# leonzheng2/Safe-Exploration-with-Simulator-in-RL-algorithms

Hardware: AMD Instinct MI355X
Metric: env-steps/sec (higher is better)
Workload: dtype f64; 1 GPU; ARS V2 iteration, 3-segment swimmer, 512 directions/GPU x 2 rollouts x H=1000 (BASELINE configs[2] per GPU); directions_total=512, directions_per_gpu=512, horizon=1000, segments=3, trajectory_capture=True, full_covariance=True, parallelism=directions sharded over 1 GPU(s), 1 all-gather/iteration, ranks_seen=1

## Files before the change

### include/swimmer_hip.h

```cpp
#ifndef SWIMMER_HIP_H
#define SWIMMER_HIP_H

#include <stdint.h>

#ifdef __cplusplus
extern "C" {
#endif

#define SW_ABI_VERSION 3
#define SW_MAX_SEGMENTS 8

#define SW_OK 0
#define SW_ERR_NULL 1
#define SW_ERR_SEGMENTS 2
#define SW_ERR_SIZE 3
#define SW_ERR_PARAM 4
#define SW_ERR_LAUNCH 5

#define SW_STATUS_OK 0
#define SW_STATUS_SINGULAR 1
#define SW_STATUS_NONFINITE 2
#define SW_STATUS_RANGE 4
#define SW_STATUS_PARAM 8

#define SW_FLAG_ROLLOUT_LANE 1
#define SW_FLAG_ROLLOUT_QUAD 2

#define SW_FLAG_MODEL_TWIN 4

typedef struct sw_params {
    int32_t n;
    int32_t flags;
    double l_i;
    double m_i;
    double k;
    double h;
    double dir_x;
    double dir_y;
} sw_params;

int sw_abi_version(void);
const char *sw_strerror(int code);
int sw_max_segments(void);

int sw_reset_f64(const sw_params *p, int64_t n_env, double *state, void *stream);

int sw_step_f64(const sw_params *p, int64_t n_env, const double *state_in,
                const double *action, double *state_out, double *reward,
                int32_t *status, void *stream);

int sw_step_residual_f64(const sw_params *p, int64_t n_env, const double *state, const double *action,
                         const double *next_ref, double *partial, void *stream);
int64_t sw_step_residual_blocks(int64_t n_env);

int sw_step_residual_pop_f64(const sw_params *base, int64_t n_cand, const double *cand, int64_t n_env,
                             const double *state, const double *action, const double *next_ref, double *partial,
                             double *value, int32_t *cand_status, void *stream);

int sw_accel_f64(const sw_params *p, int64_t n_env, const double *state,
                 const double *action, double *gdd, double *tdd, void *stream);

int sw_rollout_f64(const sw_params *p, int64_t n_roll, int32_t H, const double *policies,
                   const double *mean, const double *inv_std, const double *state0,
                   double *returns, double *traj, double *final_state, double *moments,
                   int32_t *status, void *stream);

#define SW_COST_ABS_OBS 0
#define SW_COST_MAX_ABS_THETADOT 1
int sw_safe_rollouts_f64(const sw_params *real, const sw_params *sim, int64_t n_roll, int32_t H,
                         const double *policies, int32_t cost_kind, int32_t cost_index, double sim_thresh,
                         double real_thresh, double *returns, double *traj, int32_t *first_refused,
                         int32_t *violations, int32_t *status, void *stream);

int64_t sw_moments_blocks(int64_t n_roll);

int sw_ars_rollouts_f64(const sw_params *p, int64_t dir_begin, int64_t n_dir, int32_t H,
                        const double *policy, const double *deltas, double nu,
                        const double *mean, const double *inv_std, double *returns,
                        double *traj, double *moments, int32_t *status, void *stream);

int sw_ars_gate_f64(const sw_params *sim, int64_t dir_begin, int64_t n_dir, int32_t H,
                    const double *policy, const double *deltas, double nu,
                    const double *mean, const double *inv_std, double sim_thresh,
                    int32_t *admit, double *returns, int32_t *status, void *stream);

int sw_ars_update_f64(const sw_params *p, int64_t n_dir, const double *returns,
                      const double *deltas, double *policy, double alpha, double b,
                      int64_t top_b, const double *moments, int64_t n_moment_rows,
                      double *running, int64_t n_new_states, double *mean, double *inv_std,
                      double *sigma_out, void *stream);

int sw_ars_rollouts_multi_f64(const sw_params *p, int64_t n_agent, int64_t n_dir, int32_t H,
                              const double *policy, const double *deltas, double nu,
                              const double *mean, const double *inv_std, double *returns,
                              double *moments, int32_t *status, void *stream);

int sw_ars_update_multi_f64(const sw_params *p, int64_t n_agent, int64_t n_dir, const double *returns,
                            const double *deltas, double *policy, double alpha, double b,
                            int64_t top_b, const double *moments, int64_t n_moment_rows,
                            double *running, int64_t n_new_states, double *mean, double *inv_std,
                            double *sigma_out, void *stream);

#define SW_CACLA_HIDDEN 12
#define SW_CACLA_NET_DOUBLES(n) (SW_CACLA_HIDDEN * (2 * (n) + 2) + 2 * SW_CACLA_HIDDEN + 1)
int sw_cacla_run_f64(const sw_params *p, int64_t n_agent, int32_t n_iter, int32_t train,
                     const double *gamma, const double *alpha, const double *noise, double *weights,
                     double *state, double *rewards, int32_t *actor_updates, int32_t *status, void *stream);

int sw_ars_update_gathered_f64(const sw_params *p, int64_t n_dir, const double *gathered,
// ... 72 lines not shown
```

### safe-exploration-with-simulator-in-rl-algorithms_amd/_build.py

```python
import os
import shutil
import subprocess
import tempfile
from concurrent.futures import ThreadPoolExecutor

_HERE = os.path.dirname(os.path.abspath(__file__))
CSRC = os.path.join(_HERE, "csrc")
LIB_PATH = os.environ.get("SWIMMER_HIP_LIB") or os.path.join(CSRC, "libswimmer_hip.so")
OBJ_DIR = LIB_PATH + ".obj"
SOURCES = ["swimmer_kernels.hip", "swimmer_abi.hip", "swimmer_cacla.hip", "direct_comm.cpp", "host_rng.cpp"]
FAMILIES = ["swimmer_rollout_row.hip", "swimmer_rollout_n3.hip", "swimmer_rollout_lane.hip", "swimmer_step.hip",
            "swimmer_cov.hip", "swimmer_update.hip"]
HOST_ONLY = {"host_rng.cpp"}
HEADERS = ["rlglue_env.cpp", os.path.join("..", "..", "include", "rlglue_swimmer.h"),
           "swimmer_launch.h", "swimmer_cov.h", "swimmer_device.h", "swimmer_rollout_lane.inc",
           "swimmer_rollout_quad3.inc", "swimmer_rollout_oct3.inc", "swimmer_rollout_row.inc",
           "swimmer_rollout_multi.inc", "swimmer_update.inc", "swimmer_quad3.h",
           "swimmer_oct3.h", "swimmer_row.h", "swimmer_row_fused.h", "swimmer_twin.h",
           os.path.join("..", "..", "include", "swimmer_hip.h")] + FAMILIES
HIPCC_FLAGS = ["-O3", "--offload-arch=gfx950", "-std=c++17", "-fPIC"] + os.environ.get("SWIMMER_HIPCC_EXTRA", "").split()
HOST_FLAGS = ["-O3", "-std=c++17", "-fPIC"]
LINK_LIBS = ["-ldl"]
LLVM = "/opt/rocm/lib/llvm/bin"


def _hipcc():
    exe = shutil.which("hipcc") or "/opt/rocm/bin/hipcc"
    if not os.path.exists(exe):
        raise RuntimeError("hipcc not found: the swimmer HIP library cannot be built")
    return exe


def _newer_than(path, deps):
    if not os.path.exists(path):
        return True
    t = os.path.getmtime(path)
    deps = [os.path.join(CSRC, d) for d in deps]
    return any(os.path.exists(d) and os.path.getmtime(d) > t for d in deps)


def is_stale():
    return _newer_than(LIB_PATH, SOURCES + HEADERS)


RLGLUE_LIB_PATH = os.path.join(CSRC, "librlglue_swimmer_hip.so")


def _object(src):
    return os.path.join(OBJ_DIR, os.path.splitext(src)[0] + ".o")


def _compile(src, verbose):
    flags = HOST_FLAGS + ["-x", "c++"] if src in HOST_ONLY else HIPCC_FLAGS + ["-x", "hip"]
    cmd = [_hipcc()] + flags + ["-c", os.path.join(CSRC, src), "-o", _object(src)]
    if verbose:
        print(" ".join(cmd), flush=True)
    done = subprocess.run(cmd, cwd=CSRC, capture_output=True, text=True)
    if done.returncode != 0:
        raise RuntimeError(f"hipcc failed on {src} (exit {done.returncode}):\n{done.stderr}")
    if verbose and done.stderr:
        print(done.stderr, end="", flush=True)


def build_library(force=False, verbose=False):
    if not force and not is_stale() and os.path.exists(RLGLUE_LIB_PATH):
        return LIB_PATH
    os.makedirs(OBJ_DIR, exist_ok=True)
    todo = [s for s in SOURCES if force or _newer_than(_object(s), [s] + HEADERS)]
    jobs = max(1, min(16, int(os.environ.get("MAX_JOBS", 16))))
    with ThreadPoolExecutor(max_workers=jobs) as pool:
        for _ in pool.map(lambda s: _compile(s, verbose), todo):
            pass
    cmd = ([_hipcc(), "-shared", "-fPIC", "--offload-arch=gfx950"] + [_object(s) for s in SOURCES]
           + LINK_LIBS + ["-o", LIB_PATH])
    if verbose:
        print(" ".join(cmd), flush=True)
    subprocess.check_call(cmd, cwd=CSRC)
    cmd = [_hipcc()] + HIPCC_FLAGS + ["-shared", os.path.join(CSRC, "rlglue_env.cpp"), "-L" + CSRC,
                                      "-lswimmer_hip", "-Wl,-rpath,$ORIGIN", "-o", RLGLUE_LIB_PATH]
    if verbose:
        print(" ".join(cmd), flush=True)
    subprocess.check_call(cmd, cwd=CSRC)
    return LIB_PATH


def disassemble(lib=None, raw_insn=False):
    magic = b"__CLANG_OFFLOAD_BUNDLE__"
    lines = []
    with tempfile.TemporaryDirectory() as tmp:
        fat = os.path.join(tmp, "fat.bin")
        subprocess.run([f"{LLVM}/llvm-objcopy", "-O", "binary", "--only-section=.hip_fatbin", lib or LIB_PATH, fat],
                       check=True)
        with open(fat, "rb") as f:
            blob = f.read()
        starts, at = [], blob.find(magic)
        while at >= 0:
            starts.append(at)
            at = blob.find(magic, at + 1)
        for k, (a, b) in enumerate(zip(starts, starts[1:] + [len(blob)])):
            bundle, elf = os.path.join(tmp, f"bundle{k}.bin"), os.path.join(tmp, f"gfx950_{k}.elf")
# ... 9 lines not shown
```

### safe-exploration-with-simulator-in-rl-algorithms_amd/_lib.py

```python
import ctypes
import os

import numpy as np
import torch

from . import _build

ABI_VERSION = 3
MAX_SEGMENTS = 8

ERR_NAMES = {0: "SW_OK", 1: "SW_ERR_NULL", 2: "SW_ERR_SEGMENTS", 3: "SW_ERR_SIZE",
             4: "SW_ERR_PARAM", 5: "SW_ERR_LAUNCH"}
STATUS_SINGULAR = 1
STATUS_NONFINITE = 2
STATUS_RANGE = 4
FLAG_ROLLOUT_LANE = 1
FLAG_ROLLOUT_QUAD = 2
FLAG_MODEL_TWIN = 4
COST_ABS_OBS = 0
COST_MAX_ABS_THETADOT = 1


class SwParams(ctypes.Structure):
    _fields_ = [("n", ctypes.c_int32), ("flags", ctypes.c_int32), ("l_i", ctypes.c_double),
                ("m_i", ctypes.c_double), ("k", ctypes.c_double), ("h", ctypes.c_double),
                ("dir_x", ctypes.c_double), ("dir_y", ctypes.c_double)]

    @classmethod
    def make(cls, n=3, l_i=1.0, m_i=1.0, k=10.0, h=1e-3, direction=(1.0, 0.0), flags=0):
        return cls(int(n), int(flags), float(l_i), float(m_i), float(k), float(h),
                   float(direction[0]), float(direction[1]))

    @property
    def d(self):
        return 2 * self.n + 2

    @property
    def m(self):
        return self.n - 1


class SwimmerHipError(RuntimeError):
    pass


def kernel_flags(name):
    try:
        return {"auto": 0, "lane": FLAG_ROLLOUT_LANE, "quad": FLAG_ROLLOUT_QUAD}[name]
    except KeyError:
        raise SwimmerHipError(f"rollout kernel must be 'auto', 'lane' or 'quad', not {name!r}")


_lib = None

_PROTOTYPES = {
    "sw_abi_version": (ctypes.c_int, []),
    "sw_max_segments": (ctypes.c_int, []),
    "sw_strerror": (ctypes.c_char_p, [ctypes.c_int]),
    "sw_moments_blocks": (ctypes.c_int64, [ctypes.c_int64]),
    "sw_reset_f64": (ctypes.c_int, [ctypes.c_void_p, ctypes.c_int64, ctypes.c_void_p,
                                    ctypes.c_void_p]),
    "sw_step_f64": (ctypes.c_int, [ctypes.c_void_p, ctypes.c_int64] + [ctypes.c_void_p] * 6),
    "sw_step_residual_f64": (ctypes.c_int, [ctypes.c_void_p, ctypes.c_int64] + [ctypes.c_void_p] * 5),
    "sw_step_residual_blocks": (ctypes.c_int64, [ctypes.c_int64]),
    "sw_step_residual_pop_f64": (ctypes.c_int, [ctypes.c_void_p, ctypes.c_int64, ctypes.c_void_p, ctypes.c_int64]
                                 + [ctypes.c_void_p] * 7),
    "sw_accel_f64": (ctypes.c_int, [ctypes.c_void_p, ctypes.c_int64] + [ctypes.c_void_p] * 5),
    "sw_rollout_f64": (ctypes.c_int, [ctypes.c_void_p, ctypes.c_int64, ctypes.c_int32]
                       + [ctypes.c_void_p] * 10),
    "sw_safe_rollouts_f64": (ctypes.c_int, [ctypes.c_void_p, ctypes.c_void_p, ctypes.c_int64, ctypes.c_int32,
                                            ctypes.c_void_p, ctypes.c_int32, ctypes.c_int32, ctypes.c_double,
                                            ctypes.c_double] + [ctypes.c_void_p] * 6),
    "sw_ars_rollouts_f64": (ctypes.c_int, [ctypes.c_void_p, ctypes.c_int64, ctypes.c_int64,
                                           ctypes.c_int32, ctypes.c_void_p, ctypes.c_void_p,
                                           ctypes.c_double] + [ctypes.c_void_p] * 7),
    "sw_ars_gate_f64": (ctypes.c_int, [ctypes.c_void_p, ctypes.c_int64, ctypes.c_int64, ctypes.c_int32,
                                       ctypes.c_void_p, ctypes.c_void_p, ctypes.c_double, ctypes.c_void_p,
                                       ctypes.c_void_p, ctypes.c_double] + [ctypes.c_void_p] * 4),
    "sw_ars_update_f64": (ctypes.c_int, [ctypes.c_void_p, ctypes.c_int64, ctypes.c_void_p,
                                         ctypes.c_void_p, ctypes.c_void_p, ctypes.c_double,
                                         ctypes.c_double, ctypes.c_int64, ctypes.c_void_p,
                                         ctypes.c_int64, ctypes.c_void_p, ctypes.c_int64,
                                         ctypes.c_void_p, ctypes.c_void_p, ctypes.c_void_p,
                                         ctypes.c_void_p]),
    "sw_ars_rollouts_multi_f64": (ctypes.c_int, [ctypes.c_void_p, ctypes.c_int64, ctypes.c_int64,
                                                 ctypes.c_int32, ctypes.c_void_p, ctypes.c_void_p,
                                                 ctypes.c_double] + [ctypes.c_void_p] * 6),
    "sw_ars_update_multi_f64": (ctypes.c_int, [ctypes.c_void_p, ctypes.c_int64, ctypes.c_int64,
                                               ctypes.c_void_p, ctypes.c_void_p, ctypes.c_void_p,
                                               ctypes.c_double, ctypes.c_double, ctypes.c_int64,
                                               ctypes.c_void_p, ctypes.c_int64, ctypes.c_void_p,
                                               ctypes.c_int64, ctypes.c_void_p, ctypes.c_void_p,
                                               ctypes.c_void_p, ctypes.c_void_p]),
    "sw_cacla_run_f64": (ctypes.c_int, [ctypes.c_void_p, ctypes.c_int64, ctypes.c_int32, ctypes.c_int32]
                         + [ctypes.c_void_p] * 9),
    "sw_traj_moments_f64": (ctypes.c_int, [ctypes.c_void_p, ctypes.c_int64, ctypes.c_int32,
                                           ctypes.c_void_p, ctypes.c_void_p, ctypes.c_void_p]),
    "sw_cov_acc_doubles": (ctypes.c_int64, [ctypes.c_void_p, ctypes.c_int64, ctypes.c_int32]),
    "sw_env1_create": (ctypes.c_int, [ctypes.POINTER(ctypes.c_void_p)]),
    "sw_env1_destroy": (None, [ctypes.c_void_p]),
    "sw_env1_io": (ctypes.POINTER(ctypes.c_double), [ctypes.c_void_p]),
    "sw_env1_step": (ctypes.c_int, [ctypes.c_void_p, ctypes.c_void_p, ctypes.POINTER(ctypes.c_int32)]),
    "sw_env1_accel": (ctypes.c_int, [ctypes.c_void_p, ctypes.c_void_p]),
    "sw_comm_available": (ctypes.c_int, []),
    "sw_comm_unique_id": (ctypes.c_int, [ctypes.c_void_p]),
    "sw_comm_create": (ctypes.c_int, [ctypes.POINTER(ctypes.c_void_p), ctypes.c_void_p, ctypes.c_int32,
                                      ctypes.c_int32]),
    "sw_comm_destroy": (None, [ctypes.c_void_p]),
    "sw_comm_all_gather_f64": (ctypes.c_int, [ctypes.c_void_p, ctypes.c_void_p, ctypes.c_void_p,
                                              ctypes.c_int64, ctypes.c_void_p]),
    "sw_comm_last_error": (ctypes.c_char_p, [ctypes.c_void_p]),
    "sw_issue_probe": (ctypes.c_int, [ctypes.c_int32, ctypes.c_int32, ctypes.c_void_p, ctypes.c_void_p]),
    "sw_issue_probe_grid": (ctypes.c_int, [ctypes.c_int32, ctypes.c_int32, ctypes.c_int32, ctypes.c_int32,
                                           ctypes.c_void_p, ctypes.c_void_p]),
    "sw_mt19937_uniform_pm1": (ctypes.c_int, [ctypes.c_void_p, ctypes.POINTER(ctypes.c_int32),
                                              ctypes.c_int64, ctypes.c_void_p]),
    "sw_mt19937_force_isa": (ctypes.c_int, [ctypes.c_int]),
    "sw_ars_pipeline_create": (ctypes.c_int, [ctypes.POINTER(ctypes.c_void_p)]),
    "sw_ars_pipeline_destroy": (None, [ctypes.c_void_p]),
    "sw_ars_pipeline_slots": (ctypes.c_int, []),
    "sw_ars_pipeline_next_slot": (ctypes.c_int, [ctypes.c_void_p]),
    "sw_ars_pipeline_host_slot_wait": (ctypes.c_int, [ctypes.c_void_p, ctypes.c_int]),
    "sw_ars_pipeline_sync_cov": (ctypes.c_int, [ctypes.c_void_p]),
    "sw_ars_pipeline_timing": (ctypes.c_int, [ctypes.c_void_p, ctypes.c_int]),
    "sw_ars_pipeline_rollout_ms": (ctypes.c_int, [ctypes.c_void_p,
                                                  ctypes.POINTER(ctypes.c_double),
                                                  ctypes.POINTER(ctypes.c_int64)]),
    "sw_ars_iteration_rollouts_f64": (ctypes.c_int, [ctypes.c_void_p, ctypes.c_int,
                                                     ctypes.c_void_p, ctypes.c_int64,
                                                     ctypes.c_int64, ctypes.c_int64,
                                                     ctypes.c_int32, ctypes.c_void_p,
                                                     ctypes.c_void_p, ctypes.c_void_p,
                                                     ctypes.c_double] + [ctypes.c_void_p] * 8),
# ... 98 lines not shown
```

### safe-exploration-with-simulator-in-rl-algorithms_amd/csrc/swimmer_launch.h

```cpp
#pragma once
#include <hip/hip_runtime.h>
#include <math.h>
#include <stdint.h>
#include <climits>
#include <cstdlib>
#include <type_traits>
#include <utility>

#include "../../include/swimmer_hip.h"
#include "swimmer_device.h"
#include "swimmer_twin.h"

#define SW_PIN_LOOP(PAD) asm volatile(".p2align 6\n\t.fill %0, 4, 0xbf800000" ::"n"(PAD))
#ifndef SW_OCT_UNROLL
#define SW_OCT_UNROLL 8
#endif
#ifdef SW_OCT_LOOP_PAD
constexpr int oct_loop_pad(bool, bool) { return SW_OCT_LOOP_PAD; }
#else
constexpr int oct_loop_pad(bool traj, bool mom) { return traj ? (mom ? 5 : 6) : (mom ? 6 : 2); }
#endif
#ifndef SW_QUAD_LOOP_PAD
#define SW_QUAD_LOOP_PAD 0
#endif
#ifdef SW_ROW_LOOP_PAD
constexpr int row_loop_pad(int, bool, bool) { return SW_ROW_LOOP_PAD; }
#else
constexpr int row_loop_pad(int n, bool traj, bool mom)
{
    if (n == 6 && !(traj && mom)) return traj ? 6 : 4;
    return n == 4 ? 5 : n == 5 ? 0 : n == 6 ? 5 : n == 7 ? 6 : 1;
}
#endif

#ifdef SW_MULTI_LOOP_PAD
constexpr int oct_multi_loop_pad(bool) { return SW_MULTI_LOOP_PAD; }
constexpr int quad_multi_loop_pad(bool) { return SW_MULTI_LOOP_PAD; }
constexpr int row_multi_loop_pad(int, bool) { return SW_MULTI_LOOP_PAD; }
#else
constexpr int oct_multi_loop_pad(bool) { return 11; }
constexpr int quad_multi_loop_pad(bool) { return 3; }
constexpr int row_multi_loop_pad(int n, bool mom)
{
    return n == 4 ? (mom ? 1 : 3) : n == 5 ? (mom ? 11 : 15) : n == 6 ? (mom ? 11 : 13) : n == 7 ? (mom ? 10 : 1)
                                                                                                 : (mom ? 9 : 4);
}
#endif

#ifndef SW_QUAD_UNROLL
#define SW_QUAD_UNROLL 4
#endif
#ifndef SW_TRAJ_STORE_AUX
#define SW_TRAJ_STORE_AUX 16
#endif
#ifndef SW_N3_DEFAULT_OCT
#define SW_N3_DEFAULT_OCT true
#endif

namespace {

constexpr int kWave = 64;
constexpr int kStepBlock = 256;
constexpr int kRollBlock = 64;
constexpr int kOctBlock = 128;
constexpr int kMomGroup = 16;
constexpr int64_t kQuadMaxRollouts = 16384;
constexpr int64_t kRowMaxRollouts = 8192;
constexpr int kRowBlock = 256;
constexpr int kUpdBlock = 256;
constexpr int kUpdBlockWide = 1024;
constexpr int32_t kUpdWideFrom = 1025;
constexpr int kMomBlock = 256;
constexpr int64_t kStepStreamBytes = (int64_t)256 << 20;
constexpr int kPopGroup = 8;
constexpr int64_t kPopMaxCandidates = (int64_t)65535 * kPopGroup;
constexpr double kHalfPi = 1.57079632679489661923;
constexpr double kTwinStart = 0.001;

sw::Consts make_consts(const sw_params *p)
{
    return sw::consts_of(p->n, p->l_i, p->m_i, p->k, p->h, p->dir_x, p->dir_y);
}

sw::TwinConsts make_twin_consts(const sw_params *p)
{
    return sw::TwinConsts{p->l_i, p->m_i, p->k, p->h, p->dir_x, p->dir_y};
}

inline bool is_twin(const sw_params *p) { return (p->flags & SW_FLAG_MODEL_TWIN) != 0; }

int validate_params(const sw_params *p)
{
    if (!p) return SW_ERR_NULL;
    if (p->n < 2 || p->n > SW_MAX_SEGMENTS) return SW_ERR_SEGMENTS;
    if (p->flags & ~(SW_FLAG_ROLLOUT_LANE | SW_FLAG_ROLLOUT_QUAD | SW_FLAG_MODEL_TWIN)) return SW_ERR_PARAM;
    if (!(p->l_i > 0.0) || !(p->m_i > 0.0) || !isfinite(p->l_i) || !isfinite(p->m_i) ||
        !isfinite(p->k) || !isfinite(p->h) || !isfinite(p->dir_x) || !isfinite(p->dir_y))
        return SW_ERR_PARAM;
    return SW_OK;
}

int check_params(const sw_params *p)
{
    (void)hipGetLastError();
    return validate_params(p);
}

int launch_status()
{
    return hipGetLastError() == hipSuccess ? SW_OK : SW_ERR_LAUNCH;
}

template <class F> void with_bools(F &&f) { f(); }
template <class F, class... Rest> void with_bools(F &&f, bool b, Rest... rest)
{
    if (b)
        with_bools([&](auto... cs) { f(std::true_type{}, cs...); }, rest...);
    else
        with_bools([&](auto... cs) { f(std::false_type{}, cs...); }, rest...);
}

template <int LO, int HI, class F, class... Bools> bool with_n(int n, F &&f, Bools... bools)
{
    if constexpr (LO > HI) {
        return false;
    } else {
        if (n != LO) return with_n<LO + 1, HI>(n, f, bools...);
        with_bools([&](auto... cs) { f(std::integral_constant<int, LO>{}, cs...); }, bools...);
        return true;
    }
}

template <int XOR>
__device__ __forceinline__ double swizzle_xor_f64(double v)
{
    static_assert(XOR > 0 && XOR < 32, "ds_swizzle bit-mask mode reaches lanes within 32");
    constexpr int kPattern = 0x1f | (XOR << 10);
    int lo = __double2loint(v), hi = __double2hiint(v);
    lo = __builtin_amdgcn_ds_swizzle(lo, kPattern);
    hi = __builtin_amdgcn_ds_swizzle(hi, kPattern);
    return __hiloint2double(hi, lo);
}

template <int XOR>
__device__ __forceinline__ void gate_store(double ret, int code, bool owner, int64_t r, double thr,
                                           double *__restrict__ returns, int32_t *__restrict__ status,
                                           int32_t *__restrict__ admit)
{
    const double partner = swizzle_xor_f64<XOR>(ret);
    if (owner) {
        if (returns) returns[r] = ret;
        if (status) status[r] = code;
        if ((r & 1) == 0) admit[r >> 1] = (!(ret <= thr) && !(partner <= thr)) ? 1 : 0;
    }
}

template <int D, int M, bool ARS>
__device__ __forceinline__ void load_policy_row(const double *__restrict__ pl,
                                                const double *__restrict__ dl, double sgn, double nu,
                                                const double *__restrict__ mean,
                                                const double *__restrict__ inv_std, double c12,
                                                int seg, const int (&cols)[D], double (&V)[D],
                                                double &nbias)
{
    const int a_up = (seg >= 1) ? seg - 1 : 0, a_dn = (seg <= M - 1) ? seg : M - 1;
    double pu[D], pd[D], du[D], dd[D], is[D], mn[D];
#pragma unroll
    for (int j = 0; j < D; ++j) {
        pu[j] = pl[a_up * D + cols[j]];
        pd[j] = pl[a_dn * D + cols[j]];
    }
    if (ARS) {
#pragma unroll
        for (int j = 0; j < D; ++j) {
            du[j] = dl[a_up * D + cols[j]];
            dd[j] = dl[a_dn * D + cols[j]];
        }
    }
// ... 103 lines not shown
```

### safe-exploration-with-simulator-in-rl-algorithms_amd/csrc/swimmer_oct3.h

```cpp
#pragma once

#include "swimmer_quad3.h"

namespace sw {

constexpr double kTripSlack = 0.04;

constexpr int kDppRowRor8 = 0x128;

template <int CTRL>
__device__ __forceinline__ double dpp_row_f64(double v)
{
    int lo = __double2loint(v), hi = __double2hiint(v);
    lo = __builtin_amdgcn_mov_dpp(lo, CTRL, 0xf, 0xf, true);
    hi = __builtin_amdgcn_mov_dpp(hi, CTRL, 0xf, 0xf, true);
    return __hiloint2double(hi, lo);
}

struct OctLane {
    double kvw0, kvw1, kvw2;
    double ka0, ka1, ka2;
    double kt1, kt2;
    double t1, t2, t12;
    double d0, d12, d1, d2;
// ... 104 lines not shown
{
    const Quad3Lane L = quad3_lane(seg);
    const double sg = cosine ? -1.0 : 1.0;
    OctLane O;
    O.kvw0 = sg * (L.vw0 * C.l);
    O.kvw1 = sg * (L.vw1 * C.l);
    O.kvw2 = sg * (L.vw2 * C.l);
    O.ka0 = sg * L.a0;
    O.ka1 = sg * L.a1;
    O.ka2 = sg * L.a2;
    O.kt1 = sg * L.t1;
    O.kt2 = sg * L.t2;
    O.t1 = L.t1;
    O.t2 = L.t2;
    O.t12 = L.t12;
    O.d0 = L.d0;
    O.d12 = L.d12;
    O.d1 = L.d1;
    O.d2 = L.d2;
    return O;
}

struct OctGeo {
    double u, v, u1, v1, u2, v2;
    double cc1, cc2, cc12;
    double f1, f2;
};

__device__ __forceinline__ OctGeo oct3_geometry(const OctTrig &T)
{
    OctGeo G;
    const double r = T.r, z = r * r;
    double p = fma3(T.k[0], z, T.k[1]);
    p = fma3(p, z, T.k[2]);
    p = fma3(p, z, T.k[3]);
    p = fma3(p, z, T.k[4]);
    p = fma3(p, z, T.k[5]);
    p = fma3(p, z, T.k[6]);
    const double X = __builtin_fma(T.selS, r, T.selC);
    G.u = __builtin_fma(X * z, p, X);
    G.v = dpp_row_f64<kDppRowRor8>(G.u);
    G.u1 = dpp_f64<kDppNext1>(G.u);
    G.v1 = dpp_f64<kDppNext1>(G.v);
    G.u2 = dpp_f64<kDppNext2>(G.u);
    G.v2 = dpp_f64<kDppNext2>(G.v);
    G.cc1 = __builtin_fma(G.u, G.u1, G.v * G.v1);
    G.cc2 = __builtin_fma(G.u, G.u2, G.v * G.v2);
    G.cc12 = __builtin_fma(G.u1, G.u2, G.v1 * G.v2);
    G.f1 = __builtin_fma(G.v, G.u1, -G.u * G.v1);
    G.f2 = __builtin_fma(G.v, G.u2, -G.u * G.v2);
    return G;
}

__device__ __forceinline__ double oct3_dynamics(const Consts &C, const OctLane &O, const OctGeo &G,
                                                double &Pu, double Pv, double &thd, double w1, double w2,
                                                double tq_scaled)
{
    double g = __builtin_fma(Pv, G.v, -Pu * G.u);
    g = __builtin_fma(O.kvw0, thd, g);
    g = __builtin_fma(O.kvw1 * G.cc1, w1, g);
    g = __builtin_fma(O.kvw2 * G.cc2, w2, g);
    const double g1 = dpp_f64<kDppNext1>(g), g2 = dpp_f64<kDppNext2>(g);
    const double su = __builtin_fma(g2, G.u2, __builtin_fma(g1, G.u1, g * G.u));
    double cent = __builtin_fma(O.kt1 * (w1 * w1), G.f1, tq_scaled);
    cent = __builtin_fma(O.kt2 * (w2 * w2), G.f2, cent);
    double fric = O.ka0 * g;
    fric = __builtin_fma(O.ka1 * G.cc1, g1, fric);
    fric = __builtin_fma(O.ka2 * G.cc2, g2, fric);
    double r0 = __builtin_fma(-C.six_k_m, fric, cent);
    r0 = __builtin_fma(C.kl_m, thd, r0);
    const double r1 = dpp_f64<kDppNext1>(r0), r2 = dpp_f64<kDppNext2>(r0);
    const double a = O.t1 * G.cc1, b = O.t2 * G.cc2, e = O.t12 * G.cc12;
    const double c00 = __builtin_fma(-e, e, O.d12);
    const double c01 = __builtin_fma(b, e, -a * O.d2);
    const double c02 = __builtin_fma(a, e, -b * O.d1);
    const double det = __builtin_fma(O.d0, c00, __builtin_fma(a, c01, b * c02));
    const double num = __builtin_fma(c00, r0, __builtin_fma(c01, r1, c02 * r2));
    const double tdd = num * rcp_f64_1n(det);
    Pu = __builtin_fma(C.h_kl_nm, su, Pu);
    thd = __builtin_fma(C.h, tdd, thd);
    return det;
}

}
```

### safe-exploration-with-simulator-in-rl-algorithms_amd/csrc/swimmer_rollout_n3.hip

```cpp
#include "swimmer_cov.h"
#include "swimmer_quad3.h"
#include "swimmer_oct3.h"

namespace {

template <bool ARS, bool TRAJ, bool MOM>
__global__ void __launch_bounds__(kRollBlock)
rollout_quad3_kernel(sw::Consts C, int64_t n_roll, int32_t H, const double *__restrict__ policies,
                     const double *__restrict__ deltas, int64_t dir_begin, double nu,
                     const double *__restrict__ mean, const double *__restrict__ inv_std,
                     const double *__restrict__ state0, double *__restrict__ returns,
                     double *__restrict__ traj, double *__restrict__ final_state,
                     double *__restrict__ moments, int32_t *__restrict__ status, SideJob side)
{
#define SW_GATE_BODY 0
#include "swimmer_rollout_quad3.inc"
#undef SW_GATE_BODY
}

__global__ void __launch_bounds__(kRollBlock)
ars_gate_quad3_kernel(sw::Consts C, int64_t n_roll, int32_t H, const double *__restrict__ policies,
                      const double *__restrict__ deltas, int64_t dir_begin, double nu,
                      const double *__restrict__ mean, const double *__restrict__ inv_std, double gate_thr,
                      int32_t *__restrict__ admit, double *__restrict__ returns, int32_t *__restrict__ status,
                      SideJob side)
{
    constexpr bool ARS = true, TRAJ = false, MOM = false;
    const double *const state0 = nullptr;
    double *const traj = nullptr;
    double *const final_state = nullptr;
    double *const moments = nullptr;
#define SW_GATE_BODY 1
#include "swimmer_rollout_quad3.inc"
#undef SW_GATE_BODY
}

template <bool ARS, bool TRAJ, bool MOM>
__global__ void __launch_bounds__(kOctBlock)
rollout_oct3_kernel(sw::Consts C, int64_t n_roll, int32_t H, const double *__restrict__ policies,
                    const double *__restrict__ deltas, int64_t dir_begin, double nu,
                    const double *__restrict__ mean, const double *__restrict__ inv_std,
                    const double *__restrict__ state0, double *__restrict__ returns,
                    double *__restrict__ traj, double *__restrict__ final_state,
                    double *__restrict__ moments, int32_t *__restrict__ status, SideJob side)
{
#define SW_GATE_BODY 0
#include "swimmer_rollout_oct3.inc"
#undef SW_GATE_BODY
}

__global__ void __launch_bounds__(kOctBlock)
ars_gate_oct3_kernel(sw::Consts C, int64_t n_roll, int32_t H, const double *__restrict__ policies,
                     const double *__restrict__ deltas, int64_t dir_begin, double nu,
                     const double *__restrict__ mean, const double *__restrict__ inv_std, double gate_thr,
                     int32_t *__restrict__ admit, double *__restrict__ returns, int32_t *__restrict__ status,
                     SideJob side)
{
    constexpr bool ARS = true, TRAJ = false, MOM = false;
    const double *const state0 = nullptr;
    double *const traj = nullptr;
    double *const final_state = nullptr;
    double *const moments = nullptr;
#define SW_GATE_BODY 1
#include "swimmer_rollout_oct3.inc"
#undef SW_GATE_BODY
}

#define SW_MULTI_N 3
template <bool MOM>
__global__ void __launch_bounds__(kRollBlock)
ars_multi_quad3_kernel(sw::Consts C, int64_t n_roll, int32_t H, sw_launch::MultiArgs all, double nu, SideJob side)
{
    constexpr bool ARS = true, TRAJ = false;
#include "swimmer_rollout_multi.inc"
#define SW_GATE_BODY 0
#include "swimmer_rollout_quad3.inc"
#undef SW_GATE_BODY
}

template <bool MOM>
__global__ void __launch_bounds__(kOctBlock)
ars_multi_oct3_kernel(sw::Consts C, int64_t n_roll, int32_t H, sw_launch::MultiArgs all, double nu, SideJob side)
{
    constexpr bool ARS = true, TRAJ = false;
#include "swimmer_rollout_multi.inc"
#define SW_GATE_BODY 0
#include "swimmer_rollout_oct3.inc"
#undef SW_GATE_BODY
}
#undef SW_MULTI_N

__device__ __forceinline__ double oct_sel(bool take, double a, double b) { return take ? a : b; }

template <bool TRAJ, bool VIOL>
__global__ void __launch_bounds__(kOctBlock)
safe_rollout_oct3_kernel(sw::Consts Cr, sw::Consts Cs, double tq_ratio, int64_t n_roll, int32_t H,
                         const double *__restrict__ policies, int32_t cost_kind, int32_t cost_index,
                         double sim_thresh, double real_thresh, double *__restrict__ returns,
                         double *__restrict__ traj, int32_t *__restrict__ first_refused,
                         int32_t *__restrict__ violations, int32_t *__restrict__ status)
{
    __builtin_amdgcn_s_setprio(3);
    constexpr int D = 8, M = 2;
    const int tid = threadIdx.x, lane = tid & (kWave - 1), wave = tid / kWave;
    const int q = lane & 3;
    const int seg = (q == 3) ? 0 : q;
    const bool cosine = (lane & 8) != 0;
    const int64_t r_raw = (int64_t)blockIdx.x * kMomGroup + wave * 8 + (lane >> 4) * 2 + ((lane >> 2) & 1);
    const bool valid = r_raw < n_roll;
    const int64_t r = valid ? r_raw : n_roll - 1;
    const sw::OctLane Or = sw::oct3_lane(Cr, seg, cosine), Os = sw::oct3_lane(Cs, seg, cosine);
    const int cth = 2 + 2 * seg, cthd = 3 + 2 * seg;
    const int seg1 = (seg + 1) % 3, seg2 = (seg + 2) % 3;
    const int cols[D] = {0, 1, cth, cthd, 2 + 2 * seg1, 3 + 2 * seg1, 2 + 2 * seg2, 3 + 2 * seg2};
    double V[D], nbias;
    load_policy_row<D, M, false>(policies + r * (M * D), nullptr, 1.0, 0.0, nullptr, nullptr, Cr.c12, seg, cols, V,
                                 nbias);
    const double VPu = cosine ? V[1] : V[0], VPv = cosine ? V[0] : V[1];

    const bool segA = !cosine && q < 3;
    bool own_pu = false, own_th = false, own_thd = false;
    if (cost_kind == SW_COST_MAX_ABS_THETADOT) {
        own_thd = segA;
    } else if (cost_index == 0) {
        own_pu = !cosine && q == 0;
    } else if (cost_index == 1) {
        own_pu = cosine && q == 0;
    } else {
        const bool mine = segA && seg == ((cost_index - 2) >> 1);
        own_thd = mine && ((cost_index - 2) & 1);
        own_th = mine && !((cost_index - 2) & 1);
    }
    const bool owner = own_pu || own_th || own_thd;

    double th = kHalfPi, thd = 0.0, Pu = 0.0, Pv = 0.0;
    const uint32_t kDrop = 0xfffffff0u;
    const bool rec = !cosine && q < 3;
    const uint32_t off_th = rec ? (uint32_t)(((int64_t)cth * n_roll + r) * 8) : kDrop;
    const uint32_t off_thd = rec ? (uint32_t)(((int64_t)cthd * n_roll + r) * 8) : kDrop;
    const uint32_t off_g = (q == 0) ? (uint32_t)(((int64_t)(cosine ? 1 : 0) * n_roll + r) * 8) : kDrop;
    const uint32_t slab = (uint32_t)(D * n_roll * 8);
    const __amdgpu_buffer_rsrc_t trs = __builtin_amdgcn_make_buffer_rsrc(
        traj, 0, TRAJ ? (int)(uint32_t)((int64_t)H * slab) : 0, 0x00020000);
    uint32_t soff = 0;
    auto store_cell = [&](double v, uint32_t voff) {
        typedef int v2i __attribute__((ext_vector_type(2)));
        union { double d; v2i i; } u;
        u.d = v;
// ... 18 lines not shown
    asm volatile("" : "+v"(magic));
    auto all_of_rollout = [&](bool f) -> bool {
        int v = f ? 1 : 0;
        v &= __builtin_amdgcn_mov_dpp(v, 1 | (2 << 2) | (3 << 4) | (0 << 6), 0xf, 0xf, true);
        v &= __builtin_amdgcn_mov_dpp(v, 2 | (3 << 2) | (0 << 4) | (1 << 6), 0xf, 0xf, true);
        v &= __builtin_amdgcn_mov_dpp(v, sw::kDppRowRor8, 0xf, 0xf, true);
        return v != 0;
    };
    auto one_step = [&](const sw::OctGeo &Gc, sw::OctGeo &Gx) {
        double tq = __builtin_fma(VPu, Pu, Th);
        tq = __builtin_fma(VPv, Pv, tq);
        tq = __builtin_fma(V[3], thd, tq);
        tq = __builtin_fma(V[5], w1, tq);
        tq = __builtin_fma(V[7], w2, tq);
        double Pus = Pu, thds = thd;
        (void)sw::oct3_dynamics(Cs, Os, Gc, Pus, Pv, thds, w1, w2, tq * tq_ratio);
        const double ths = __builtin_fma(Cs.h, thd, th);
        const double vs = own_thd ? thds : (own_th ? ths : Pus);
        const bool safe = all_of_rollout(!owner || (fabs(vs) <= sim_thresh)) && alive;
        alive = safe;
        double Pur = Pu, thdr = thd;
        const double det_new = sw::oct3_dynamics(Cr, Or, Gc, Pur, Pv, thdr, w1, w2, tq);
        const double r_new = __builtin_fma(Cr.h, thd, A.r);
        double Th_new = __builtin_fma(hV2, thd, Th);
        Th_new = __builtin_fma(hV4, w1, Th_new);
        Th_new = __builtin_fma(hV6, w2, Th_new);
        A.r = oct_sel(safe, r_new, A.r);
        const unsigned long long outside = sw::oct3_range_test(A.r);
        Th = oct_sel(safe, Th_new, Th);
        thd = oct_sel(safe, thdr, thd);
        Pu = oct_sel(safe, Pur, Pu);
        det = oct_sel(safe, det_new, det);
        sw::oct3_keep_reduced(A, thmax, magic, designation, outside);
        th = __builtin_fma(A.kd, sw::kPio2Hi, A.r);
        Gx = sw::oct3_geometry(A);
        ret += oct_sel(safe, Pu, 0.0);
        taken += safe ? 1 : 0;
        if (VIOL) {
            const double vr = own_thd ? thd : (own_th ? th : Pu);
            const bool fine = all_of_rollout(!owner || !(fabs(vr) > real_thresh));
            over += (safe && !fine) ? 1 : 0;
        }
        if (TRAJ) {
            store_cell(th, off_th);
            store_cell(thd, off_thd);
            store_cell(Pu, off_g);
            soff += slab;
        }
        w1 = sw::dpp_f64<sw::kDppNext1>(thd);
        w2 = sw::dpp_f64<sw::kDppNext2>(thd);
        Pv = sw::dpp_row_f64<sw::kDppRowRor8>(Pu);
    };
    int32_t t = 0;
    for (; t + 2 <= H; t += 2) {
        one_step(G, Gn);
        one_step(Gn, G);
    }
    if (t < H) one_step(G, Gn);
    thmax = fmax(thmax, fabs(th));

    int code = ((det > 0.0) ? 0 : SW_STATUS_SINGULAR) |
               ((isfinite(th) && isfinite(thd) && isfinite(Pu) && isfinite(Pv)) ? 0 : SW_STATUS_NONFINITE) |
               ((thmax < sw::kAngleLimit) ? 0 : SW_STATUS_RANGE);
    code |= __builtin_amdgcn_mov_dpp(code, sw::kDppNext1, 0xf, 0xf, true) |
            __builtin_amdgcn_mov_dpp(code, sw::kDppNext2, 0xf, 0xf, true);
    code |= __builtin_amdgcn_mov_dpp(code, sw::kDppRowRor8, 0xf, 0xf, true);
    const double ret_other = sw::dpp_row_f64<sw::kDppRowRor8>(ret);
    if (valid && !cosine && q == 0) {
        const double total = __builtin_fma(Cr.dirx, ret, Cr.diry * ret_other);
        returns[r] = (code & SW_STATUS_RANGE) ? __builtin_nan("") : total;
        if (first_refused) first_refused[r] = taken;
        if (violations) violations[r] = over;
        if (status) status[r] = code;
    }
}

}

namespace sw_launch __attribute__((visibility("hidden"))) {

int launch_oct3(const sw_params *p, const RolloutPlan &plan, bool ars, int64_t n_roll, int32_t H, const RolloutArgs &a,
                hipStream_t stream, const SideWork *side)
{
    with_bools([&](auto ARS, auto TRAJ, auto MOM) {
        launch_segment_per_lane(rollout_oct3_kernel<ARS.value, TRAJ.value, MOM.value>, p, plan, n_roll, H, a, stream,
                                side);
    }, ars, a.traj != nullptr, a.moments != nullptr);
    return launch_status();
}

int launch_quad3(const sw_params *p, const RolloutPlan &plan, bool ars, int64_t n_roll, int32_t H,
                 const RolloutArgs &a, hipStream_t stream, const SideWork *side)
{
    with_bools([&](auto ARS, auto TRAJ, auto MOM) {
        launch_segment_per_lane(rollout_quad3_kernel<ARS.value, TRAJ.value, MOM.value>, p, plan, n_roll, H, a, stream,
                                side);
    }, ars, a.traj != nullptr, a.moments != nullptr);
    return launch_status();
}

int launch_gate_oct3(const sw_params *sim, const RolloutPlan &plan, int64_t n_roll, int32_t H, const RolloutArgs &a,
                     double gate_thr, int32_t *admit, hipStream_t stream)
{
    launch_gate_segment_per_lane(ars_gate_oct3_kernel, sim, plan, n_roll, H, a, gate_thr, admit, stream);
    return launch_status();
}

int launch_gate_quad3(const sw_params *sim, const RolloutPlan &plan, int64_t n_roll, int32_t H, const RolloutArgs &a,
                      double gate_thr, int32_t *admit, hipStream_t stream)
{
    launch_gate_segment_per_lane(ars_gate_quad3_kernel, sim, plan, n_roll, H, a, gate_thr, admit, stream);
    return launch_status();
}

int launch_multi_oct3(const sw_params *p, const RolloutPlan &plan, int64_t n_agent, int64_t n_roll, int32_t H,
                      const MultiArgs &a, double nu, hipStream_t stream)
{
    with_bools([&](auto MOM) {
        hipLaunchKernelGGL(ars_multi_oct3_kernel<MOM.value>, multi_grid(plan, n_agent, n_roll), dim3(plan.block), 0,
                           stream, make_consts(p), n_roll, H, a, nu, kNoSide);
    }, a.moments != nullptr);
    return launch_status();
}

int launch_multi_quad3(const sw_params *p, const RolloutPlan &plan, int64_t n_agent, int64_t n_roll, int32_t H,
                       const MultiArgs &a, double nu, hipStream_t stream)
{
    with_bools([&](auto MOM) {
        hipLaunchKernelGGL(ars_multi_quad3_kernel<MOM.value>, multi_grid(plan, n_agent, n_roll), dim3(plan.block), 0,
                           stream, make_consts(p), n_roll, H, a, nu, kNoSide);
    }, a.moments != nullptr);
    return launch_status();
}

int launch_safe_oct3(const sw_params *real, const sw_params *sim, const RolloutPlan &plan, int64_t n_roll, int32_t H,
                     const double *policies, int32_t cost_kind, int32_t cost_index, double sim_thresh,
                     double real_thresh, double *returns, double *traj, int32_t *first_refused, int32_t *violations,
                     int32_t *status, hipStream_t stream)
{
    const sw::Consts Cr = make_consts(real), Cs = make_consts(sim);
    const double tq_ratio = Cs.c12 / Cr.c12;
    with_bools([&](auto TRAJ, auto VIOL) {
        hipLaunchKernelGGL((safe_rollout_oct3_kernel<TRAJ.value, VIOL.value>), dim3(plan.rollout_blocks),
                           dim3(plan.block), 0, stream, Cr, Cs, tq_ratio, n_roll, H, policies, cost_kind, cost_index,
                           sim_thresh, real_thresh, returns, traj, first_refused, violations, status);
    }, traj != nullptr, violations != nullptr);
    return launch_status();
}

}
```

Measured before the change: 4.530 billion env-steps/s.

## Add packed oct3 rollout kernel that stores one trajectory cell per lane

Adds a new rollout kernel for the 3-segment oct layout, used by default when both trajectory capture and moments are requested. Each lane packs theta, theta-dot or position into a single value via DPP row rotation and writes one trajectory cell per step through a buffer store, accumulating moments from that same packed value. The point is to cut per-step store and moment work. A split flag restores the old path, and the new moment-reduction layout adds correctness risk.

```diff
diff --git a/include/swimmer_hip.h b/include/swimmer_hip.h
--- a/include/swimmer_hip.h
+++ b/include/swimmer_hip.h
@@ -25,6 +25,8 @@
 
 #define SW_FLAG_ROLLOUT_LANE 1
 #define SW_FLAG_ROLLOUT_QUAD 2
+
+#define SW_FLAG_CAPTURE_SPLIT 8
 
 #define SW_FLAG_MODEL_TWIN 4
 
diff --git a/safe-exploration-with-simulator-in-rl-algorithms_amd/_build.py b/safe-exploration-with-simulator-in-rl-algorithms_amd/_build.py
--- a/safe-exploration-with-simulator-in-rl-algorithms_amd/_build.py
+++ b/safe-exploration-with-simulator-in-rl-algorithms_amd/_build.py
@@ -14,8 +14,8 @@
 HOST_ONLY = {"host_rng.cpp"}
 HEADERS = ["rlglue_env.cpp", os.path.join("..", "..", "include", "rlglue_swimmer.h"),
            "swimmer_launch.h", "swimmer_cov.h", "swimmer_device.h", "swimmer_rollout_lane.inc",
-           "swimmer_rollout_quad3.inc", "swimmer_rollout_oct3.inc", "swimmer_rollout_row.inc",
-           "swimmer_rollout_multi.inc", "swimmer_update.inc", "swimmer_quad3.h",
+           "swimmer_rollout_quad3.inc", "swimmer_rollout_oct3.inc", "swimmer_rollout_octp3.inc",
+           "swimmer_rollout_row.inc", "swimmer_rollout_multi.inc", "swimmer_update.inc", "swimmer_quad3.h",
            "swimmer_oct3.h", "swimmer_row.h", "swimmer_row_fused.h", "swimmer_twin.h",
            os.path.join("..", "..", "include", "swimmer_hip.h")] + FAMILIES
 HIPCC_FLAGS = ["-O3", "--offload-arch=gfx950", "-std=c++17", "-fPIC"] + os.environ.get("SWIMMER_HIPCC_EXTRA", "").split()
diff --git a/safe-exploration-with-simulator-in-rl-algorithms_amd/_lib.py b/safe-exploration-with-simulator-in-rl-algorithms_amd/_lib.py
--- a/safe-exploration-with-simulator-in-rl-algorithms_amd/_lib.py
+++ b/safe-exploration-with-simulator-in-rl-algorithms_amd/_lib.py
@@ -17,6 +17,7 @@
 FLAG_ROLLOUT_LANE = 1
 FLAG_ROLLOUT_QUAD = 2
 FLAG_MODEL_TWIN = 4
+FLAG_CAPTURE_SPLIT = 8
 COST_ABS_OBS = 0
 COST_MAX_ABS_THETADOT = 1
 
@@ -46,9 +47,9 @@
 
 def kernel_flags(name):
     try:
-        return {"auto": 0, "lane": FLAG_ROLLOUT_LANE, "quad": FLAG_ROLLOUT_QUAD}[name]
+        return {"auto": 0, "lane": FLAG_ROLLOUT_LANE, "quad": FLAG_ROLLOUT_QUAD, "split": FLAG_CAPTURE_SPLIT}[name]
     except KeyError:
-        raise SwimmerHipError(f"rollout kernel must be 'auto', 'lane' or 'quad', not {name!r}")
+        raise SwimmerHipError(f"rollout kernel must be 'auto', 'lane', 'quad' or 'split', not {name!r}")
 
 
 _lib = None
diff --git a/safe-exploration-with-simulator-in-rl-algorithms_amd/csrc/swimmer_launch.h b/safe-exploration-with-simulator-in-rl-algorithms_amd/csrc/swimmer_launch.h
--- a/safe-exploration-with-simulator-in-rl-algorithms_amd/csrc/swimmer_launch.h
+++ b/safe-exploration-with-simulator-in-rl-algorithms_amd/csrc/swimmer_launch.h
@@ -20,6 +20,10 @@
 #else
 constexpr int oct_loop_pad(bool traj, bool mom) { return traj ? (mom ? 5 : 6) : (mom ? 6 : 2); }
 #endif
+#ifndef SW_OCTP_LOOP_PAD
+#define SW_OCTP_LOOP_PAD 4
+#endif
+constexpr int oct_packed_loop_pad() { return SW_OCTP_LOOP_PAD; }
 #ifndef SW_QUAD_LOOP_PAD
 #define SW_QUAD_LOOP_PAD 0
 #endif
@@ -93,7 +97,7 @@
 {
     if (!p) return SW_ERR_NULL;
     if (p->n < 2 || p->n > SW_MAX_SEGMENTS) return SW_ERR_SEGMENTS;
-    if (p->flags & ~(SW_FLAG_ROLLOUT_LANE | SW_FLAG_ROLLOUT_QUAD | SW_FLAG_MODEL_TWIN)) return SW_ERR_PARAM;
+    if (p->flags & ~(SW_FLAG_ROLLOUT_LANE | SW_FLAG_ROLLOUT_QUAD | SW_FLAG_MODEL_TWIN | SW_FLAG_CAPTURE_SPLIT)) return SW_ERR_PARAM;
     if (!(p->l_i > 0.0) || !(p->m_i > 0.0) || !isfinite(p->l_i) || !isfinite(p->m_i) ||
         !isfinite(p->k) || !isfinite(p->h) || !isfinite(p->dir_x) || !isfinite(p->dir_y))
         return SW_ERR_PARAM;
diff --git a/safe-exploration-with-simulator-in-rl-algorithms_amd/csrc/swimmer_oct3.h b/safe-exploration-with-simulator-in-rl-algorithms_amd/csrc/swimmer_oct3.h
--- a/safe-exploration-with-simulator-in-rl-algorithms_amd/csrc/swimmer_oct3.h
+++ b/safe-exploration-with-simulator-in-rl-algorithms_amd/csrc/swimmer_oct3.h
@@ -210,4 +210,13 @@
     return det;
 }
 
-}
+__device__ __forceinline__ double octp3_pack(double th, double thd, double Pu, bool lane3)
+{
+    int lo = __double2loint(th), hi = __double2hiint(th);
+    lo = __builtin_amdgcn_update_dpp(lo, __double2loint(thd), kDppRowRor8, 0xf, 0xc, false);
+    hi = __builtin_amdgcn_update_dpp(hi, __double2hiint(thd), kDppRowRor8, 0xf, 0xc, false);
+    const double Z = __hiloint2double(hi, lo);
+    return lane3 ? Pu : Z;
+}
+
+}
diff --git a/safe-exploration-with-simulator-in-rl-algorithms_amd/csrc/swimmer_rollout_n3.hip b/safe-exploration-with-simulator-in-rl-algorithms_amd/csrc/swimmer_rollout_n3.hip
--- a/safe-exploration-with-simulator-in-rl-algorithms_amd/csrc/swimmer_rollout_n3.hip
+++ b/safe-exploration-with-simulator-in-rl-algorithms_amd/csrc/swimmer_rollout_n3.hip
@@ -64,6 +64,18 @@
 #define SW_GATE_BODY 1
 #include "swimmer_rollout_oct3.inc"
 #undef SW_GATE_BODY
+}
+
+template <bool ARS>
+__global__ void __launch_bounds__(kOctBlock)
+rollout_octp3_kernel(sw::Consts C, int64_t n_roll, int32_t H, const double *__restrict__ policies,
+                     const double *__restrict__ deltas, int64_t dir_begin, double nu,
+                     const double *__restrict__ mean, const double *__restrict__ inv_std,
+                     const double *__restrict__ state0, double *__restrict__ returns,
+                     double *__restrict__ traj, double *__restrict__ final_state,
+                     double *__restrict__ moments, int32_t *__restrict__ status, SideJob side)
+{
+#include "swimmer_rollout_octp3.inc"
 }
 
 #define SW_MULTI_N 3
@@ -248,6 +260,12 @@
 int launch_oct3(const sw_params *p, const RolloutPlan &plan, bool ars, int64_t n_roll, int32_t H, const RolloutArgs &a,
                 hipStream_t stream, const SideWork *side)
 {
+    if (a.traj && a.moments && !(p->flags & SW_FLAG_CAPTURE_SPLIT)) {
+        with_bools([&](auto ARS) {
+            launch_segment_per_lane(rollout_octp3_kernel<ARS.value>, p, plan, n_roll, H, a, stream, side);
+        }, ars);
+        return launch_status();
+    }
     with_bools([&](auto ARS, auto TRAJ, auto MOM) {
         launch_segment_per_lane(rollout_oct3_kernel<ARS.value, TRAJ.value, MOM.value>, p, plan, n_roll, H, a, stream,
                                 side);
diff --git a/safe-exploration-with-simulator-in-rl-algorithms_amd/csrc/swimmer_rollout_octp3.inc b/safe-exploration-with-simulator-in-rl-algorithms_amd/csrc/swimmer_rollout_octp3.inc
--- /dev/null
+++ b/safe-exploration-with-simulator-in-rl-algorithms_amd/csrc/swimmer_rollout_octp3.inc
@@ -0,0 +1,160 @@
+    side_flag(side);
+    if (blockIdx.x >= side.first_cov_block) {
+        side_cov_tile<8, kOctBlock>(side);
+        return;
+    }
+    __builtin_amdgcn_s_setprio(3);
+    constexpr int D = 8, M = 2;
+    const int tid = threadIdx.x, lane = tid & (kWave - 1), wave = tid / kWave;
+    const int q = lane & 3;
+    const int seg = (q == 3) ? 0 : q;
+    const bool cosine = (lane & 8) != 0;
+    const int64_t r_raw = (int64_t)blockIdx.x * kMomGroup + wave * 8 + (lane >> 4) * 2 + ((lane >> 2) & 1);
+    const bool valid = r_raw < n_roll;
+    const int64_t r = valid ? r_raw : n_roll - 1;
+    const sw::OctLane O = sw::oct3_lane(C, seg, cosine);
+    const int cth = 2 + 2 * seg, cthd = 3 + 2 * seg;
+
+    const int seg1 = (seg + 1) % 3, seg2 = (seg + 2) % 3;
+    const int cols[D] = {0, 1, cth, cthd, 2 + 2 * seg1, 3 + 2 * seg1, 2 + 2 * seg2, 3 + 2 * seg2};
+    double V[D], nbias;
+    load_policy_row<D, M, ARS>(ARS ? policies : policies + r * (M * D),
+                               ARS ? deltas + (dir_begin + (r >> 1)) * (M * D) : nullptr,
+                               (r & 1) ? -1.0 : 1.0, nu, mean, inv_std, C.c12, seg, cols, V, nbias);
+    const double VPu = cosine ? V[1] : V[0], VPv = cosine ? V[0] : V[1];
+
+    double gdx = 0.0, gdy = 0.0, th = kHalfPi, thd = 0.0;
+    if (state0) {
+        gdx = state0[r];
+        gdy = state0[n_roll + r];
+        th = state0[(int64_t)cth * n_roll + r];
+        thd = state0[(int64_t)cthd * n_roll + r];
+    }
+    double Pu = cosine ? gdy : gdx, Pv = cosine ? gdx : gdy;
+
+    const bool lane3 = q == 3;
+    const int column = lane3 ? (cosine ? 1 : 0) : (cosine ? cthd : cth);
+    const double shift = (!cosine && !lane3) ? kHalfPi : 0.0;
+    const uint32_t voff = (uint32_t)(((int64_t)column * n_roll + r) * 8);
+    const uint32_t slab = (uint32_t)(D * n_roll * 8);
+    const __amdgpu_buffer_rsrc_t trs = __builtin_amdgcn_make_buffer_rsrc(
+        traj, 0, (int)(uint32_t)((int64_t)H * slab), 0x00020000);
+    uint32_t soff = 0;
+    auto store_cell = [&](double v) {
+        typedef int v2i __attribute__((ext_vector_type(2)));
+        union { double d; v2i i; } u;
+        u.d = v;
+        __builtin_amdgcn_raw_buffer_store_b64(u.i, trs, (int)voff, (int)soff, SW_TRAJ_STORE_AUX);
+    };
+
+    const int designation = cosine ? 1 : 0;
+    double thmax = 0.0, det = 1.0;
+    sw::OctTrig A;
+    A.r = th;
+    A.kd = 0.0;
+    sw::oct3_renorm(A, designation, thmax);
+    double m1 = 0.0, m2 = 0.0;
+    double w1 = sw::dpp_f64<sw::kDppNext1>(thd), w2 = sw::dpp_f64<sw::kDppNext2>(thd);
+    double Th = __builtin_fma(V[2], th, nbias);
+    Th = __builtin_fma(V[4], sw::dpp_f64<sw::kDppNext1>(th), Th);
+    Th = __builtin_fma(V[6], sw::dpp_f64<sw::kDppNext2>(th), Th);
+    const double hV2 = C.h * V[2], hV4 = C.h * V[4], hV6 = C.h * V[6];
+    sw::OctGeo G = sw::oct3_geometry(A), Gn;
+    double magic = 6755399441055744.0;
+    asm volatile("" : "+v"(magic));
+    auto one_step = [&](const sw::OctGeo &Gc, sw::OctGeo &Gx) {
+        A.r = __builtin_fma(C.h, thd, A.r);
+        const unsigned long long outside = sw::oct3_range_test(A.r);
+        double tq = __builtin_fma(VPu, Pu, Th);
+        tq = __builtin_fma(VPv, Pv, tq);
+        tq = __builtin_fma(V[3], thd, tq);
+        tq = __builtin_fma(V[5], w1, tq);
+        tq = __builtin_fma(V[7], w2, tq);
+        Th = __builtin_fma(hV2, thd, Th);
+        Th = __builtin_fma(hV4, w1, Th);
+        Th = __builtin_fma(hV6, w2, Th);
+        sw::oct3_keep_reduced(A, thmax, magic, designation, outside);
+        Gx = sw::oct3_geometry(A);
+        det = sw::oct3_dynamics(C, O, Gc, Pu, Pv, thd, w1, w2, tq);
+        const double Z = sw::octp3_pack(__builtin_fma(A.kd, sw::kPio2Hi, A.r), thd, Pu, lane3);
+        const double X = Z - shift;
+        m1 += X;
+        m2 = __builtin_fma(X, X, m2);
+        store_cell(Z);
+        soff += slab;
+        w1 = sw::dpp_f64<sw::kDppNext1>(thd);
+        w2 = sw::dpp_f64<sw::kDppNext2>(thd);
+        Pv = sw::dpp_row_f64<sw::kDppRowRor8>(Pu);
+    };
+    int32_t t = 0;
+    SW_PIN_LOOP(oct_packed_loop_pad());
+    for (; t + 8 <= H; t += 8) {
+        one_step(G, Gn);
+        one_step(Gn, G);
+        one_step(G, Gn);
+        one_step(Gn, G);
+        one_step(G, Gn);
+        one_step(Gn, G);
+        one_step(G, Gn);
+        one_step(Gn, G);
+    }
+    for (; t + 4 <= H; t += 4) {
+        one_step(G, Gn);
+        one_step(Gn, G);
+        one_step(G, Gn);
+        one_step(Gn, G);
+    }
+    for (; t + 2 <= H; t += 2) {
+        one_step(G, Gn);
+        one_step(Gn, G);
+    }
+    if (t < H) one_step(G, Gn);
+    if (H > 0) th = __builtin_fma(A.kd, sw::kPio2Hi, A.r);
+    thmax = fmax(thmax, fabs(th));
+
+    int code = ((det > 0.0) ? 0 : SW_STATUS_SINGULAR) |
+               ((isfinite(th) && isfinite(thd) && isfinite(Pu) && isfinite(Pv)) ? 0 : SW_STATUS_NONFINITE) |
+               ((thmax < sw::kAngleLimit) ? 0 : SW_STATUS_RANGE);
+    code |= __builtin_amdgcn_mov_dpp(code, sw::kDppNext1, 0xf, 0xf, true) |
+            __builtin_amdgcn_mov_dpp(code, sw::kDppNext2, 0xf, 0xf, true);
+    code |= __builtin_amdgcn_mov_dpp(code, sw::kDppRowRor8, 0xf, 0xf, true);
+    const double sg_other = sw::dpp_row_f64<sw::kDppRowRor8>(m1);
+    if (valid && !cosine && lane3) {
+        const double total = __builtin_fma(C.dirx, m1, C.diry * sg_other);
+        returns[r] = (code & SW_STATUS_RANGE) ? __builtin_nan("") : total;
+        if (status) status[r] = code;
+    }
+    if (final_state && valid) {
+        if (!cosine && q < 3) {
+            final_state[(int64_t)cth * n_roll + r] = th;
+            final_state[(int64_t)cthd * n_roll + r] = thd;
+        }
+        if (q == 0) final_state[(int64_t)(cosine ? 1 : 0) * n_roll + r] = Pu;
+    }
+    {
+        __shared__ double shm[kOctBlock / kWave][16][2];
+        if (!valid) m1 = m2 = 0.0;
+#pragma unroll
+        for (int k = 0; k < 3; ++k) {
+            const int off = (k == 0) ? 4 : (k == 1 ? 16 : 32);
+            m1 += __shfl_xor(m1, off, kWave);
+            m2 += __shfl_xor(m2, off, kWave);
+        }
+        if (lane < 16) {
+            shm[wave][lane][0] = m1;
+            shm[wave][lane][1] = m2;
+        }
+        __syncthreads();
+        if (tid < 3) {
+            double *row = moments + (int64_t)blockIdx.x * (2 * D);
+            row[2 + 2 * tid] = shm[0][tid][0] + shm[1][tid][0];
+            row[D + 2 + 2 * tid] = shm[0][tid][1] + shm[1][tid][1];
+            row[3 + 2 * tid] = shm[0][8 + tid][0] + shm[1][8 + tid][0];
+            row[D + 3 + 2 * tid] = shm[0][8 + tid][1] + shm[1][8 + tid][1];
+            if (tid < 2) {
+                const int src = 3 + tid * 8;
+                row[tid] = shm[0][src][0] + shm[1][src][0];
+                row[D + tid] = shm[0][src][1] + shm[1][src][1];
+            }
+        }
+    }
```

Measured after the change: 4.676 billion env-steps/s, median of 6. +3.2%, better.
